# muzishen/IMAGHarmony

Hardware: AMD Instinct MI355X
Metric: 1024^2 SDXL images/sec (30 DDIM steps, PNS N seeds) (higher is better)
Workload: dtype bf16

## Files before the change

### imagharmony_amd/csrc/api.hip

```cpp
#include <stdarg.h>
#include <stdio.h>
#include <string.h>

#include <vector>

#include "../../include/imh.h"
#include "imh_common.h"
#include "imh_kernels.h"

namespace imh {

static thread_local char g_err[512] = "";

void set_error(const char* fmt, ...) {
    va_list ap;
    va_start(ap, fmt);
    vsnprintf(g_err, sizeof(g_err), fmt, ap);
    va_end(ap);
}

int experimental_refused(const char* what) {
    set_error("%s is compiled only with -DIMH_EXPERIMENTAL (IMH_EXPERIMENTAL=1 python -m imagharmony_amd.build): measured, not selected by any "
              "tuning.json entry or default mode", what);
    return IMH_ERR_ARG;
// ... 11 lines not shown
    GemmParams p;
    p.X = a->X; p.W = a->W; p.Y = a->Y; p.partial = a->partial; p.bias = a->bias; p.rowadd = a->rowadd;
    p.residual = a->residual; p.ln_s = a->ln_s; p.ln_c = a->ln_c; p.ln_eps = a->ln_eps;
    p.ln_stats = a->ln_stats; p.ln_stats_out = a->ln_stats_out; p.ln_slots = a->ln_slots; p.ln_slots_out = a->ln_slots_out;
    p.gn_out = a->gn_out; p.gn_nblk = a->gn_nblk; p.gn_hw = a->gn_hw;
    p.gn_tab = a->gn_tab; p.gn_silu = a->gn_silu; p.X2 = a->X2; p.Cin1 = a->X2 ? a->Cin1 : a->Cin;
    p.gn_src.partial = a->gn_part; p.gn_src.partial2 = a->gn_part2; p.gn_src.gamma = a->gn_gamma; p.gn_src.beta = a->gn_beta;
    p.gn_src.eps = a->gn_eps; p.gn_src.groups = a->gn_groups; p.gn_src.C = a->Cin; p.gn_src.C1 = a->gn_part2 ? a->gn_pC1 : a->Cin;
    p.gn_src.HW = a->H * a->Wd; p.gn_src.nblk = a->gn_pnblk; p.gn_src.sub = a->gn_psub; p.gn_src.npart = a->gn_pnpart;
    p.gn_src.nblk2 = a->gn_pnblk2; p.gn_src.sub2 = a->gn_psub2; p.gn_src.npart2 = a->gn_pnpart2; p.gn_src.dtype_f16 = a->dtype == IMH_DT_F16;
    p.Yt = a->Yt; p.yt_col0 = a->yt_col0; p.ldyt = a->ldyt;
    p.M = a->M; p.N = a->N; p.K = a->K;
    p.ldx = a->ldx; p.ldw = a->ldw; p.ldy = a->ldy; p.ldr = a->ldr; p.ldra = a->ldra > 0 ? a->ldra : a->N;
    p.rows_per_batch = a->rows_per_batch; p.splits = a->splits; p.flags = a->flags;
    p.H = a->H; p.Wd = a->Wd; p.Cin = a->Cin; p.Ho = a->Ho; p.Wo = a->Wo; p.stride = a->stride; p.up = a->up; p.pad_lo = a->pad == 1 ? 0 : 1;
    p.px = p.py = 1; p.tmx = p.tny = 0; p.xcd = a->xcd;
    p.pf_ptr = a->pf_ptr; p.pf_bytes = a->pf_bytes;
    p.early_res = g_ws_early;
    return p;
}

static int do_gemm_dual(const imh_gemm_args* a, const imh_gemm_args* b, hipStream_t s) {
    if (!a || !b || !a->X || !a->W || !a->Y || !b->X || !b->W || !b->Y) { set_error("gemm_dual: null pointer argument"); return IMH_ERR_ARG; }
    if (a->conv || b->conv || a->dtype != b->dtype) { set_error("gemm_dual: both problems must be plain GEMMs of one dtype"); return IMH_ERR_ARG; }
    int bm = a->bm, bn = a->bn;
    if (bm != 24128 && (bm <= 0 || bn <= 0 || bm > 128)) { bm = 128; bn = 64; }
    for (const imh_gemm_args* g : {a, b}) {
        if ((g->flags & (IMH_GF_LN_ROW | IMH_GF_LN_COL)) && (!g->ln_s || !g->ln_c || !(g->ln_eps > 0.f))) {
            set_error("gemm_dual: folded LayerNorm needs ln_s / ln_c / ln_eps > 0"); return IMH_ERR_ARG;
        }
// ... 12 lines not shown
    if ((p.flags & (IMH_GF_LN_ROW | IMH_GF_LN_COL)) && (!p.ln_s || !p.ln_c || !(p.ln_eps > 0.f))) { set_error("gemm: folded LayerNorm needs ln_s / ln_c / ln_eps > 0"); return IMH_ERR_ARG; }
    if ((p.flags & IMH_GF_LN_ROW) && (p.flags & IMH_GF_LN_COL)) { set_error("gemm: IMH_GF_LN_ROW and IMH_GF_LN_COL are exclusive"); return IMH_ERR_ARG; }
    if (!(p.flags & (IMH_GF_LN_ROW | IMH_GF_LN_COL))) p.ln_stats = nullptr;
    if (p.ln_stats && (p.ln_slots <= 0 || p.K % p.ln_slots)) { set_error("gemm: ln_slots=%d must divide K=%d", p.ln_slots, p.K); return IMH_ERR_ARG; }
    int bm = a->bm, bn = a->bn;
    if (bm <= 0 || bn <= 0 || p.splits <= 0) {
        int hb, hn, hs;
        gemm_pick_config(p.M, p.N, p.K, &hb, &hn, &hs);
        if (bm <= 0) bm = hb;
        if (bn <= 0) bn = hn;
        if (p.splits <= 0) p.splits = p.partial ? hs : 1;
    }
    if ((p.flags & IMH_GF_VT_PERM) && p.splits == 1) bn = 128;
    if (a->conv) {
        if (p.stride != 1 && p.stride != 2) { set_error("conv3x3: stride must be 1 or 2"); return IMH_ERR_ARG; }
        if (p.up != 0 && p.up != 1) { set_error("conv3x3: up must be 0 or 1"); return IMH_ERR_ARG; }
        if (a->pad != 0 && a->pad != 1) { set_error("conv3x3: pad must be 0 or 1"); return IMH_ERR_ARG; }
        if (a->pad == 1) {
            if (p.stride != 2 || p.up || p.H < 2 || p.Wd < 2) {
                set_error("conv3x3: pad mode 1 needs stride 2, up 0 and an input of at least 2 x 2 (stride=%d up=%d H=%d W=%d)", p.stride, p.up, p.H, p.Wd);
                return IMH_ERR_ARG;
            }
            if (bm == 7128 || bm == 7564 || bm == 7328 || bm == 7428 || bm == 7256 || bm == 7356 || bm == 8256 || bm == 9128 || bm == 9256 ||
                bm == 26256) {
                set_error("conv3x3: pad mode 1 is not implemented by variant %d x %d", bm, bn);
                return IMH_ERR_ARG;
            }
        }
        const int Hv = p.H << p.up, Wv = p.Wd << p.up;
        const int span = a->pad == 1 ? 1 : 2;
        if (p.Ho != (Hv + span - 3) / p.stride + 1 || p.Wo != (Wv + span - 3) / p.stride + 1 || p.Ho <= 0 || p.Wo <= 0) {
            set_error("conv3x3: output size %dx%d inconsistent with input %dx%d up=%d stride=%d pad=%d", p.Ho, p.Wo, p.H, p.Wd, p.up, p.stride, a->pad);
// ... 138 lines not shown
    if (key == 0) { g_attn_force_nw = value; return IMH_OK; }
    if (key == 1) {
#ifdef IMH_EXPERIMENTAL
        return 1;
#else
        return 0;
#endif
    }
    if (key == 2) { g_xcd_mode = value; return IMH_OK; }
    if (key == 3) { g_xattn_mode = value; return IMH_OK; }
    if (key == 4) { g_attn_mode = value; return IMH_OK; }
    if (key == 5) { g_halo_mode = value; return IMH_OK; }
    if (key == 7) { g_w16_pf = value; return IMH_OK; }
    if (key == 9) { g_w16_form = value; return IMH_OK; }
    if (key == 10) { g_f32_exact = value; return IMH_OK; }
    if (key == 6) { g_ws_early = value; return IMH_OK; }
    set_error("debug_set: unknown key %d", key);
    return IMH_ERR_ARG;
}
const char* imh_last_error(void) { return g_err; }

int imh_gemm(const imh_gemm_args* a, void* stream) { return do_gemm(a, (hipStream_t)stream); }
int imh_gemm_dual(const imh_gemm_args* a, const imh_gemm_args* b, void* stream) { return do_gemm_dual(a, b, (hipStream_t)stream); }
int imh_gemm_pick_config(int M, int N, int K, int* bm, int* bn, int* splits) {
    if (!bm || !bn || !splits) { set_error("pick_config: null output"); return IMH_ERR_ARG; }
    gemm_pick_config(M, N, K, bm, bn, splits);
    return IMH_OK;
}
size_t imh_gemm_workspace_bytes(int M, int N, int splits) { return gemm_workspace_bytes(M, N, splits); }
int imh_gemm_stats_slot_width(int bm, int bn) { return gemm_stats_slot_width(bm, bn); }
// ... 118 lines not shown
```

### imagharmony_amd/csrc/gemm.hip

```cpp
#include "imh_common.h"
#include "imh_kernels.h"
#include "imh_gemm_epilogue.h"
#include <algorithm>
#include <type_traits>

namespace imh {

int g_xcd_mode = 0;


template <typename T, int BM, int BN, bool CONV, int LN>
__device__ __forceinline__ void gemm_body(const GemmParams& p, const int bid, const int z) {
    constexpr int FM = BM / 32;
    constexpr int FN = BN / 32;
    constexpr int RX = BM / 32;
    constexpr int RW = BN / 32;
    constexpr int XT_BYTES = BM * GEMM_ROW_BYTES;
    constexpr int WT_BYTES = BN * GEMM_ROW_BYTES;
    constexpr int STAGE = XT_BYTES + WT_BYTES;
    typedef typename Vec<T>::v8 v8;

    extern __shared__ __attribute__((aligned(16))) unsigned char smem[];

    const int tid = threadIdx.x;
// ... 375 lines not shown
int gemm_gn_block_rows(int bm, int bn) {
    if ((bm == 1464 || bm == 2464) && bn == 160) return 32;
    if ((bm == 24128 || bm == 23256 || bm == 22128) && bn == 160) return 64;
    if (bm == 7128 || bm == 7328 || bm == 7428) return 32;
    if (bm == 7564) return 16;
    if (bm == 7256 || bm == 7356) return 64;
    return 0;
}

size_t gemm_workspace_bytes(int M, int N, int splits) {
    return splits > 1 ? (size_t)splits * M * N * sizeof(float) : 0;
}

int gemm_launch(GemmParams p, int dtype, int conv, int bm, int bn, hipStream_t stream) {
    if (p.K % GEMM_BK != 0 || p.K <= 0) { set_error("gemm: K=%d must be a positive multiple of 64", p.K); return IMH_ERR_SHAPE; }
    if (conv && (p.Cin % GEMM_BK != 0 || p.K != 9 * p.Cin)) { set_error("conv3x3: Cin=%d must be a multiple of 64 and K=9*Cin", p.Cin); return IMH_ERR_SHAPE; }
    if (!conv && ((p.ldx & 7) || (p.ldw & 7))) { set_error("gemm: ldx/ldw must be multiples of 8 elements"); return IMH_ERR_SHAPE; }
    if (p.M <= 0 || p.N <= 0) { set_error("gemm: empty problem M=%d N=%d", p.M, p.N); return IMH_ERR_SHAPE; }
    if ((p.flags & GF_GEGLU) && (p.N & 15)) { set_error("geglu: N must be a multiple of 16"); return IMH_ERR_SHAPE; }
    if (p.splits < 1) p.splits = 1;
    if (p.splits > 1 && !p.partial) { set_error("gemm: split-K needs a workspace"); return IMH_ERR_WORKSPACE; }
    if (p.rowadd && p.rows_per_batch <= 0) { set_error("gemm: rowadd needs rows_per_batch"); return IMH_ERR_ARG; }
    if ((p.flags & (GF_LN_ROW | GF_LN_COL)) && !p.ln_stats) {
        set_error("gemm: the folded LayerNorm takes the token rows' statistics from ln_stats (imh_lnstats.h: the epilogue of the GEMM that "
                  "wrote the rows, or IMH_EW_ROW_STATS); there is no in-loop E[x^2] - mean^2 form");
        return IMH_ERR_ARG;
    }
    if ((p.flags & (GF_LN_ROW | GF_LN_COL)) && (p.splits > 1 || (bm >= 256 && !((bm == 1464 || bm == 2464 || bm == 24128 || bm == 23256 || bm == 22128 || bm == 26256) && (p.flags & GF_LN_ROW))) || conv)) {
        set_error("gemm: folded LayerNorm needs a plain 64/128 tile or a wave-specialised variant (row form), splits == 1, no conv (bm=%d splits=%d conv=%d)", bm, p.splits, conv);
        return IMH_ERR_ARG;
    }
    if (p.ln_stats_out) {
        const int w = gemm_stats_slot_width(bm, bn);
        if (w == 0 || p.N % w || p.ln_slots_out != p.N / w || conv || p.splits > 1 || (p.flags & (GF_GEGLU | GF_VT_PERM | GF_OUT_F32))) {
            set_error("gemm: ln_stats_out needs a variant with a statistics epilogue (slot width %d for %dx%d), N %% width == 0, "
                      "ln_slots_out == N / width, a plain output (N=%d slots=%d flags=%d splits=%d conv=%d)", w, bm, bn, p.N, p.ln_slots_out, p.flags, p.splits, conv);
            return IMH_ERR_ARG;
        }
    }
    if (p.gn_out) {
        const int rows = gemm_gn_block_rows(bm, bn);
        const bool halo = bm >= 7000 && bm < 8000;
        if (rows == 0 || p.N % 10 || p.N % (halo ? bn : 80) || p.gn_hw <= 0 || p.gn_hw % rows || p.M % p.gn_hw || p.gn_nblk != p.gn_hw / rows ||
            p.splits > 1 || (p.flags & (GF_GEGLU | GF_VT_PERM | GF_OUT_F32 | GF_LN_ROW | GF_LN_COL)) ||
            (halo && (p.Ho % (rows * 4 / 16) || p.Wo % 16))) {
            set_error("gemm: gn_out needs a variant with a GroupNorm epilogue (%d rows per block for %dx%d), N a multiple of 10 and of the tile "
                      "width, whole tiles, gn_nblk == gn_hw / rows (N=%d hw=%d nblk=%d M=%d flags=%d)", rows, bm, bn, p.N, p.gn_hw, p.gn_nblk, p.M, p.flags);
            return IMH_ERR_ARG;
        }
    }
    {
        const bool halo = bm >= 7000 && bm < 8000;
        const bool ws = bm == 1464 || bm == 2464 || bm == 24128 || bm == 23256 || bm == 22128;
        if ((p.gn_tab || p.gn_src.partial) && !(conv && halo)) {
            set_error("gemm: the fused GroupNorm front end (gn_tab / gn_part) is a form of the LDS-halo conv3x3 (variant %d)", bm);
            return IMH_ERR_ARG;
        }
        if (p.gn_src.partial && (p.gn_tab || !gn_src_ok(p.gn_src))) {
// ... 33 lines not shown
```

### imagharmony_amd/csrc/gemm_ring.hip

```cpp
#include "imh_common.h"
#include "imh_kernels.h"
#include "imh_gemm_epilogue.h"
#include "imh_lnstats.h"
#include <type_traits>

namespace imh {

int g_ws_early = 1;

template <int N> __device__ __forceinline__ void wait_vmcnt() {
    asm volatile("s_waitcnt vmcnt(%0)" ::"n"(N) : "memory");
}

template <typename T, int BM, int BN, int WM, int WN, int S, bool CONV>
__global__ __launch_bounds__(64 * WM * WN, 1) void gemm_ring_kernel(const GemmParams p) {
    constexpr int NW = WM * WN;
    constexpr int NT = 64 * NW;
    constexpr int TM = BM / WM, TN = BN / WN;
    constexpr int FM = TM / 16, FN = TN / 16;
    constexpr int RPR = NW * 8;
    constexpr int RX = BM / RPR, RW = BN / RPR;
    constexpr int LP = RX + RW;
    constexpr int XT_BYTES = BM * GEMM_ROW_BYTES;
    constexpr int WT_BYTES = BN * GEMM_ROW_BYTES;
// ... 7 lines not shown

    const int tid = threadIdx.x;
    const int lane = tid & 63;
    const int wave = __builtin_amdgcn_readfirstlane(tid >> 6);
    const int wm = wave / WN, wn = wave % WN;

    int m0, n0;
    if (!xcd_tile<BM, BN>(p, blockIdx.x, m0, n0)) return;

    const int nkt = p.K / GEMM_BK;
    const int z = blockIdx.y;
    const int per = (nkt + p.splits - 1) / p.splits;
    const int kt0 = z * per;
    const int kt1 = min(nkt, kt0 + per);
    const int nt = max(0, kt1 - kt0);

    const unsigned char* zero = g_zero_page;
    const int srow = wave * 8 + (lane >> 3);

    const unsigned char* xbase[RX];
    int xstep[RX];
    int cb[RX], coy[RX], cox[RX];
    bool cvalid[RX];
#pragma unroll
    for (int i = 0; i < RX; ++i) {
        const int row = i * RPR + srow;
        const int c = stage_chunk_x(row, lane);
        const int m = m0 + row;
        const bool ok = m < p.M;
        if (!CONV) {
// ... 16 lines not shown
        const int row = i * RPR + srow;
        const int c = stage_chunk_w(row, lane, FN);
        const int n = n0 + row;
        const bool ok = n < p.N;
        wbase[i] = ok ? (const unsigned char*)p.W + ((size_t)n * p.ldw) * sizeof(T) + c * 16 : zero + c * 16;
        wstep[i] = ok ? GEMM_BK * (int)sizeof(T) : 0;
    }
    const int cpt = CONV ? p.Cin / GEMM_BK : 1;

    auto stage = [&](int slot, int kt) {
        unsigned char* xs = smem + slot * STAGE;
        unsigned char* ws = xs + XT_BYTES;
        if (CONV) {
            const int tap = kt / cpt;
            const int ct = kt - tap * cpt;
            const int ky = tap / 3, kx = tap - ky * 3;
            const int Hv = p.H << p.up, Wv = p.Wd << p.up;
#pragma unroll
            for (int i = 0; i < RX; ++i) {
                const int c = stage_chunk_x(i * RPR + srow, lane);
                const int iy = coy[i] * p.stride + ky - p.pad_lo;
                const int ix = cox[i] * p.stride + kx - p.pad_lo;
                const bool ok = cvalid[i] && iy >= 0 && iy < Hv && ix >= 0 && ix < Wv;
                const size_t pix = ((size_t)cb[i] * p.H + (iy >> p.up)) * p.Wd + (ix >> p.up);
                const unsigned char* src = ok
                    ? (const unsigned char*)p.X + (pix * p.Cin + (size_t)ct * GEMM_BK) * sizeof(T) + c * 16
                    : zero + c * 16;
                glds16(src, xs + (i * RPR + wave * 8) * GEMM_ROW_BYTES);
            }
        } else {
#pragma unroll
// ... 60 lines not shown
        if (m >= p.M || nb >= p.N) continue;
        float v[4 * FN];
#pragma unroll
        for (int j = 0; j < FN; ++j)
#pragma unroll
            for (int r = 0; r < 4; ++r) v[j * 4 + r] = acc[i][j][r];
        if (p.splits > 1) {
            float* o = p.partial + ((size_t)z * p.M + m) * p.N + nb;
            if (nb + 4 * FN <= p.N && (p.N & 3) == 0) {
#pragma unroll
                for (int q0 = 0; q0 < 4 * FN; q0 += 4) *(f32x4*)(o + q0) = f32x4{v[q0], v[q0 + 1], v[q0 + 2], v[q0 + 3]};
            } else {
#pragma unroll
                for (int q = 0; q < 4 * FN; ++q) if (nb + q < p.N) o[q] = v[q];
            }
        } else {
            epilogue_store<T, FN>(p, v, m, nb);
        }
    }
    if (z == 0) tail_prefetch(p.pf_ptr, p.pf_bytes, blockIdx.x, gridDim.x, tid, blockDim.x);
}

template <typename T, int BM, int BN, bool CONV>
__global__ __launch_bounds__(512, 2) void gemm_kg2_kernel(const GemmParams p) {
    constexpr int FM = BM / 32, FN = BN / 32;
    constexpr int RX = BM / 32, RW = BN / 32;
    constexpr int XT_BYTES = BM * GEMM_ROW_BYTES;
    constexpr int WT_BYTES = BN * GEMM_ROW_BYTES;
    constexpr int STAGE = XT_BYTES + WT_BYTES;
    constexpr int GROUP_BYTES = 2 * STAGE;
// ... 198 lines not shown
    const int tid = threadIdx.x;
    const int lane = tid & 63;
    const int wave = __builtin_amdgcn_readfirstlane(tid >> 6);

#if WS_TIMING
    const unsigned long long ts_entry = __builtin_amdgcn_s_memrealtime();
#endif
    int m0, n0;
    if (!xcd_tile<BM, BN>(p, bid, m0, n0)) return;
    const int nkt = p.K / GEMM_BK;
    const int z = blockIdx.y;
    const int per = (nkt + p.splits - 1) / p.splits;
    const int kt0 = z * per;
    const int kt1 = min(nkt, kt0 + per);
    const int nt = max(0, kt1 - kt0);

    if (wave >= NC) {
        const int pw = wave - NC;
        const unsigned char* zero = g_zero_page;
        const unsigned char* base[LP];
        const unsigned char* base2[KX > 0 ? KX : 1];
        const int kt_x2 = (!CONV && p.X2) ? p.Cin1 / GEMM_BK : 0x7fffffff;
        int step[LP];
        int cb[KX > 0 ? KX : 1], coy[KX > 0 ? KX : 1], cox[KX > 0 ? KX : 1];
        bool cvalid[KX > 0 ? KX : 1];
#pragma unroll
        for (int k = 0; k < LP; ++k) {
            const int r = (k * NL + pw) * 8 + (lane >> 3);
            if (k < KX) {
                const int c = stage_chunk_x(r, lane);
// ... 18 lines not shown
                const int c = stage_chunk_w(row, lane, FN);
                const int n = n0 + row;
                const bool ok = n < p.N;
                base[k] = ok ? (const unsigned char*)p.W + ((size_t)n * p.ldw) * sizeof(T) + c * 16 : zero + c * 16;
                step[k] = ok ? GEMM_BK * (int)sizeof(T) : 0;
            }
        }
        const int cpt = CONV ? p.Cin / GEMM_BK : 1;
        auto issue = [&](int slot, int kt) {
            unsigned char* st = smem + slot * STAGE;
            int ky = 0, kx = 0, ct = 0;
            if (CONV) {
                const int tap = kt / cpt;
                ct = kt - tap * cpt;
                ky = tap / 3; kx = tap - ky * 3;
            }
#pragma unroll
            for (int k = 0; k < LP; ++k) {
                unsigned char* dst = st + (k * NL + pw) * 8 * GEMM_ROW_BYTES;
                if (CONV && k < KX) {
                    const int r = (k * NL + pw) * 8 + (lane >> 3);
                    const int c = stage_chunk_x(r, lane);
                    const int Hv = p.H << p.up, Wv = p.Wd << p.up;
                    const int iy = coy[k] * p.stride + ky - p.pad_lo;
                    const int ix = cox[k] * p.stride + kx - p.pad_lo;
                    const bool ok = cvalid[k] && iy >= 0 && iy < Hv && ix >= 0 && ix < Wv;
                    const size_t pix = ((size_t)cb[k] * p.H + (iy >> p.up)) * p.Wd + (ix >> p.up);
                    const unsigned char* src = ok
                        ? (const unsigned char*)p.X + (pix * p.Cin + (size_t)ct * GEMM_BK) * sizeof(T) + c * 16
                        : zero + c * 16;
// ... 141 lines not shown
    }
    if (nt > 0) mm(K1);
#if WS_TIMING
    const unsigned long long ts_loop1 = __builtin_amdgcn_s_memrealtime();
    if (bid == 0 && wave == 0 && lane == 0 && p.pf_ptr) {
        unsigned long long* dbg = (unsigned long long*)p.pf_ptr;
        dbg[0] = tacc[0]; dbg[1] = tacc[1]; dbg[2] = tacc[2]; dbg[3] = nt;
    }
    if (wave == 0 && lane == 0 && p.pf_ptr && p.pf_bytes == 0xfeed) {
        unsigned long long* dbg = (unsigned long long*)p.pf_ptr + 8 + (size_t)bid * 4;
        dbg[0] = ts_entry; dbg[1] = ts_loop0; dbg[2] = ts_loop1; dbg[3] = 0;
    }
#endif

    const int nb = n0 + wn * TN + (lane >> 4) * 4 * FN;
    float lnpre[8 * FN];
    const bool have_pre = ln_preload<4 * FN>(p, nb, lnpre);
    EpiPre<4 * FN> pre;
    pre.ok = !p.rowadd && !p.residual && p.splits == 1 && epilogue_fast<T, 4 * FN>(p, nb);
    if (pre.ok && p.bias) ldv<T, 4 * FN>((const T*)p.bias + nb, pre.bias);
    LnArgs<4 * FN> ln;
    float st_s[FM], st_q[FM];
    constexpr int GNV = (4 * FN) % 10 == 0 ? 4 * FN : 10;
    GnAcc<GNV> gna;
    gn_zero(gna);
    if constexpr (LN == 2) {
        const f32x2s* ex = (const f32x2s*)(smem + S * STAGE);
#pragma unroll
        for (int q = 0; q < 4 * FN; ++q) {
            const f32x2s mr = ex[wn * TN + (lane >> 4) * 4 * FN + q];
            ln.cm[q] = mr[0]; ln.cr[q] = mr[1];
        }
    }
    if constexpr (LN == 1) {
        const float* ex = (const float*)(smem + S * STAGE);
// ... 158 lines not shown
#pragma unroll
        for (int j = 0; j < FN; ++j)
#pragma unroll
            for (int r = 0; r < 4; ++r) v[j * 4 + r] = acc[i][j][r];
        if (p.splits > 1) {
            float* o = p.partial + ((size_t)z * p.M + m) * p.N + nb;
            if (nb + 4 * FN <= p.N && (p.N & 3) == 0) {
#pragma unroll
                for (int q0 = 0; q0 < 4 * FN; q0 += 4) *(f32x4*)(o + q0) = f32x4{v[q0], v[q0 + 1], v[q0 + 2], v[q0 + 3]};
            } else {
#pragma unroll
                for (int q = 0; q < 4 * FN; ++q) if (nb + q < p.N) o[q] = v[q];
            }
        } else {
            if constexpr (LN == 1) { ln.mean = st_s[i]; ln.rstd = st_q[i]; }
            epilogue_store_pre<T, FN>(p, v, m, nb, lnpre, have_pre, LN != 0 ? &ln : nullptr, LN != 0 ? nullptr : &pre, lane,
                                      (LN == 0 && (4 * FN) % 10 == 0) ? &gna : nullptr, i == 0);
        }
    }
    if constexpr (LN == 0 && (4 * FN) % 10 == 0) {
        if (p.gn_out && p.splits == 1) {
            const int mw = m0 + wm * TM;
            if (mw < p.M) gn_emit<4 * FN>(p.gn_out, p.gn_nblk, p.N / 10, mw / p.gn_hw, (mw % p.gn_hw) / TM, nb, gna, FM, lane);
        }
    }
}

template <typename T, int BM, int BN, int CM, int CN, int S, int NP, bool CONV, int LN, int OCC = 1>
__global__ __launch_bounds__(64 * (CM * CN + NP), OCC == 1 ? 1 : OCC * (CM * CN + NP) / 4) void gemm_ws_kernel(const GemmParams p) {
    extern __shared__ __attribute__((aligned(16))) unsigned char smem[];
    gemm_ws_body<T, BM, BN, CM, CN, S, NP, CONV, LN>(p, blockIdx.x, gridDim.x, smem);
#if WS_TIMING
    if (threadIdx.x == 0 && p.pf_ptr && p.pf_bytes == 0xfeed) {
        asm volatile("s_waitcnt vmcnt(0)" ::: "memory");
        ((unsigned long long*)p.pf_ptr)[8 + (size_t)blockIdx.x * 4 + 3] = __builtin_amdgcn_s_memrealtime();
    }
#endif
}
// ... 124 lines not shown
```

### imagharmony_amd/csrc/imh_gemm_epilogue.h

```cpp
#pragma once
#include "imh_common.h"
#include "imh_kernels.h"
#include "imh_lnstats.h"

namespace imh {

template <int BM, int BN>
__device__ __forceinline__ bool xcd_tile(const GemmParams& p, int b, int& m0, int& n0) {
    if (p.px == 0) {
        m0 = (b / p.tny) * BM;
        n0 = (b % p.tny) * BN;
        return m0 < p.M;
    }
    const int xcd = b & 7, s = b >> 3;
    const int xi = xcd / p.py, yi = xcd - xi * p.py;
    const int ms = s / p.tny, ns = s - ms * p.tny;
    m0 = (xi * p.tmx + ms) * BM;
    n0 = (yi * p.tny + ns) * BN;
    return ms < p.tmx && m0 < p.M && n0 < p.N;
}

inline void xcd_partition(GemmParams& p, int bm, int bn, int* grid) {
    const int tm = (p.M + bm - 1) / bm, tn = (p.N + bn - 1) / bn;
    if (g_xcd_mode == 1) { p.px = 0; p.py = 1; p.tmx = tm; p.tny = tn; *grid = tm * tn; return; }
    int bpx = 8, bpy = 1;
    double best = 1e300;
    const int cand[4][2] = {{8, 1}, {4, 2}, {2, 4}, {1, 8}};
    for (auto& c : cand) {
        const int tmx = (tm + c[0] - 1) / c[0], tny = (tn + c[1] - 1) / c[1];
        const double waste = (double)(tmx * c[0]) * (tny * c[1]) / ((double)tm * tn);
        const double cost = ((double)c[1] * p.M + (double)c[0] * p.N) * waste * waste;
        if (cost < best) { best = cost; bpx = c[0]; bpy = c[1]; }
    }
    const int forced = g_xcd_mode ? g_xcd_mode : p.xcd;
    if (forced >= 2 && forced <= 5) { bpx = cand[forced - 2][0]; bpy = cand[forced - 2][1]; }
    p.px = bpx; p.py = bpy;
    p.tmx = (tm + bpx - 1) / bpx;
    p.tny = (tn + bpy - 1) / bpy;
    *grid = 8 * p.tmx * p.tny;
}

enum : int {
    GF_GEGLU = 1,
    GF_ACT_GELU = 2,
    GF_ACT_SILU = 4,
    GF_VT_PERM = 8,
    GF_OUT_F32 = 16,
    GF_LN_ROW = 32,
    GF_LN_COL = 64,
};

template <typename T, int CNT>
__device__ __forceinline__ void ldv(const T* p, float* o) {
    static_assert(CNT % 2 == 0, "vector epilogue works on even column counts");
// ... 243 lines not shown
```

### imagharmony_amd/csrc/imh_kernels.h

```cpp
#pragma once
#include <hip/hip_runtime.h>
#include <stddef.h>
#include "imh_gntable.h"

namespace imh {

struct GemmParams {
    const void* X;
    const void* W;
    void* Y;
    float* partial;
    const void* bias;
    const void* rowadd;
    const void* residual;
    const float* ln_s;
    const float* ln_c;
    float ln_eps;
    const float* ln_stats;
    float* ln_stats_out;
    int ln_slots, ln_slots_out;
    float* gn_out;
    int gn_nblk, gn_hw;
    const float* gn_tab;
    int gn_silu;
    GnTabSrc gn_src;
    const void* X2;
    int Cin1;
    void* Yt;
    int yt_col0, ldyt;
    int M, N, K;
    int ldx, ldw, ldy, ldr, ldra;
    int rows_per_batch;
    int splits;
    int flags;
    int H, Wd, Cin, Ho, Wo, stride, up, pad_lo;
    int px, py, tmx, tny;
    int xcd;
    const void* pf_ptr;
    unsigned pf_bytes;
    int early_res;
};

void gemm_pick_config(int M, int N, int K, int* bm, int* bn, int* splits);
size_t gemm_workspace_bytes(int M, int N, int splits);
int gemm_stats_slot_width(int bm, int bn);
int gemm_gn_block_rows(int bm, int bn);
int gemm_launch(GemmParams p, int dtype, int conv, int bm, int bn, hipStream_t stream);
int gemm_dual_launch(GemmParams a, GemmParams b, int dtype, int bm, int bn, hipStream_t stream);
int gemm_w16_launch(const GemmParams& p, int dtype, hipStream_t stream);

// ... 29 lines not shown
    const float* ln_stats;
    int ln_slots;
    int C, ldx, ldw;
    int split;
};
int xattn_launch(const XAttnParams& p, int dtype, hipStream_t stream);
extern int g_attn_force_nw;
extern int g_xattn_mode;
extern int g_w16_pf;
extern int g_w16_form;
extern int g_f32_exact;
extern int g_attn_mode;
extern int g_xcd_mode;
extern int g_halo_mode;
extern int g_ws_early;

struct SmallAttnParams {
    const void* Q; const void* K; const void* V; void* O;
    int B, H, Lq, Lk, dq, dv;
    int ldq, ldk, ldv, ldo;
    float scale;
};
int attention_small_launch(const SmallAttnParams& p, int dtype, hipStream_t stream);

struct NormParams {
    const void* x;
    void* y;
    const void* gamma;
    const void* beta;
    float* partial;
// ... 51 lines not shown
```

### imagharmony_amd/ctx.py

```python
import ctypes as C
import json
import os

import torch

from . import lib as L

_DT = {torch.bfloat16: L.IMH_DT_BF16, torch.float16: L.IMH_DT_F16}
_TUNING_PATH = os.environ.get("IMH_TUNING_PATH") or os.path.join(os.path.dirname(os.path.abspath(__file__)), "tuning.json")


_TUNING_CACHE = None


def _load_tuning():
    global _TUNING_CACHE
    if _TUNING_CACHE is None:
        _TUNING_CACHE = _read_tuning()
    return _TUNING_CACHE


def _read_tuning():
    try:
        with open(_TUNING_PATH) as f:
            raw = json.load(f)
        extra = os.environ.get("IMH_TUNING_OVERRIDE")
        if extra:
            raw.update(json.loads(extra))
        return {tuple(int(v) for v in k.split(",")): tuple(cfg) for k, cfg in raw.items()}
    except (OSError, ValueError):
        return {}


class GnStats:
    __slots__ = ("t", "nblk", "sub", "npart", "C")

    def __init__(self, t, nblk, sub, npart, C_):
        self.t, self.nblk, self.sub, self.npart, self.C = t, int(nblk), int(sub), int(npart), int(C_)


class GnSpec:
    def __init__(self, stats, gamma, beta, groups, eps):
        self.srcs = list(stats) if isinstance(stats, (list, tuple)) else [stats]
        self.gamma, self.beta, self.groups, self.eps = gamma, beta, int(groups), float(eps)
        self.C = sum(g.C for g in self.srcs)

# ... 119 lines not shown
    def _p(t):
        return None if t is None else t.data_ptr()

    def _chk(self, t, name, dtype=None):
        if t is None:
            return
        if t.device != self.device and not (t.device.type == "cuda" and t.device.index == (self.device.index or 0)):
            raise L.ImhError(f"{name}: tensor on {t.device}, context on {self.device}")
        if t.dtype != (dtype or self.dtype):
            raise L.ImhError(f"{name}: dtype {t.dtype}, expected {dtype or self.dtype}")

    _WS = (1464, 2464, 24128, 23256, 22128)
    _W16 = (26256,)
    _PP = (8256, 9128, 9256)
    _HALO = (7128, 7564, 7328, 7428, 7256, 7356)

    @classmethod
    def _variant_ok(cls, bm, sp, flags, conv, stride, ln_pre, M=0, N=0, extras=False, pad=0):
        plain = bm <= 128
        if pad and (not conv or bm in cls._HALO + cls._PP + cls._W16):
            return False
        if bm in cls._W16:
            return not conv and sp == 1 and bool(flags & L.GF_LN_ROW) and not flags & ~(L.GF_LN_ROW | L.GF_GEGLU) and bool(ln_pre) \
                and not extras and M % 256 == 0 and N % 320 == 0
        if bm in cls._HALO:
            return bool(conv) and stride == 1 and not flags & (L.GF_LN_ROW | L.GF_LN_COL | L.GF_VT_PERM)
        if flags & (L.GF_VT_PERM | L.GF_LN_COL):
            return plain and (sp == 1 or not flags & L.GF_LN_COL)
        if flags & L.GF_LN_ROW:
            return sp == 1 and not conv and (plain or bm in cls._WS)
# ... 163 lines not shown
        else:
            L.check(self.lib.imh_gemm_dual(C.byref(pair[0]), C.byref(pair[1]), self.stream()), descr)
        if own is not None:
            self.free(own[0])
        return o1, o2

    def conv_fuses_gn(self, M, N, K, stride=1, up=0, cfg=None):
        bm, bn, sp = cfg or self._config(M, N, K, 1, 0, stride=stride, up=up)
        if bm not in self._HALO or stride != 1 or up:
            return False
        ph = 4 if bm == 7564 else (16 if bm in (7256, 7356) else 8)
        S = (6 if ph == 16 else 9) if bn == 80 else (3 if bm in (7328, 7356) else (4 if bm == 7428 else 2))
        lds = 2 * (((ph + 2) * 18 + 7) // 8) * 8 * 128 + S * bn * 128 + (K // 9) * 8
        return lds <= 160 * 1024

    def conv3x3(self, x, w, bias=None, stride=1, up=0, residual=None, rowadd=None, ldra=0, out=None, cfg=None,
                descr="conv3x3", gn_groups=0, gn=None, x2=None, pad=0):
        self._chk(x, descr + ".x"); self._chk(w, descr + ".w")
        B, H, W, C1 = x.shape
        Cin = C1 + (x2.shape[-1] if x2 is not None else 0)
        Cout = w.shape[0]
        Hv, Wv = H << up, W << up
        if pad and (stride != 2 or up or gn is not None or x2 is not None):
            raise L.ImhError(f"{descr}: pad mode 1 is a plain stride-2 conv (no upsampling, fused GroupNorm or second source)")
        Ho, Wo = ((Hv - 2) // 2 + 1, (Wv - 2) // 2 + 1) if pad else ((Hv - 1) // stride + 1, (Wv - 1) // stride + 1)
        M, N, K = B * Ho * Wo, Cout, 9 * Cin
        if not x.is_contiguous() or not w.is_contiguous() or w.shape[1] != K:
            raise L.ImhError(f"{descr}: x must be contiguous NHWC and w packed [Cout, 9*Cin]")
        if x2 is not None:
            self._chk(x2, descr + ".x2")
            if tuple(x2.shape[:3]) != (B, H, W) or not x2.is_contiguous() or C1 % 64 or x2.shape[-1] % 64:
                raise L.ImhError(f"{descr}: x2 must be contiguous NHWC over the same pixels, both channel counts multiples of 64")
# ... 411 lines not shown
```

### imagharmony_amd/lib.py

```python
import ctypes as C
import os

_HERE = os.path.dirname(os.path.abspath(__file__))
_EXP_PATH = os.path.join(_HERE, "..", "tools", "tmp_libs", "libimh_hip_experimental.so")
LIB_PATH = os.environ.get("IMH_LIB_PATH") or (_EXP_PATH if os.environ.get("IMH_EXPERIMENTAL") == "1" else os.path.join(_HERE, "libimh_hip.so"))

ABI_VERSION = 11
IMH_DT_BF16, IMH_DT_F16 = 0, 1
GF_GEGLU, GF_ACT_GELU, GF_ACT_SILU, GF_VT_PERM, GF_OUT_F32, GF_LN_ROW, GF_LN_COL = 1, 2, 4, 8, 16, 32, 64
OP_GEMM, OP_ATTN, OP_GROUPNORM, OP_LAYERNORM, OP_EW, OP_ATTN_SMALL, OP_GEMM_DUAL, OP_XATTN = 0, 1, 2, 3, 4, 5, 6, 7
GN_ALL, GN_STATS, GN_TABLE, GN_APPLY, GN_TABLE_APPLY = 0, 1, 2, 3, 4
(EW_TIMESTEP, EW_SILU, EW_CONCAT, EW_CONV_IN, EW_CFG_STEP, EW_CAST_F32, EW_ADD, EW_STEP_SET, EW_CFG_RESCALE, EW_SOFTMAX,
 EW_ROW_STATS, EW_STEP_ROW) = range(12)

EXP_VARIANTS = {(4064, 64), (4064, 128), (4128, 64), (5256, 320), (6128, 320), (6064, 160), (7064, 160), (256, 128), (256, 256), (22128, 160),
                (3128, 128), (24128, 128), (9256, 320), (7564, 320), (7564, 160), (7328, 160), (7428, 160), (7256, 80)}


def experimental():
    return load().imh_debug_set(1, 0) == 1


def variant_built(cfg):
    return (int(cfg[0]), int(cfg[1])) not in EXP_VARIANTS or experimental()
# ... 140 lines not shown
```

### imagharmony_amd/unet.py

```python
import math
import os
from dataclasses import dataclass
from typing import Dict, Tuple

import torch
import torch.nn as nn

from . import lib as L
from .attention_processor import AttnProcessor2_0, IPAttnProcessor2_0, _b, _vkey, _w
from .ctx import Ctx, GnSpec


FOLD_LAYERNORM = True
LN_STATS_HANDOVER = os.environ.get("IMH_LN_STATS", "1") != "0"
GN_STATS_HANDOVER = os.environ.get("IMH_GN_STATS", "1") != "0"
GN_FUSE = os.environ.get("IMH_GN_FUSE", "1") != "0"
GN_TABLE_FOLD = os.environ.get("IMH_GN_TABLE_FOLD", "1") != "0"


class Feat:
    __slots__ = ("t", "gs")

    def __init__(self, t, gs=None):
        self.t, self.gs = t, gs

    def stats(self, ctx, groups):
        if self.gs is None:
            B, C_ = self.t.shape[0], self.t.shape[-1]
            self.gs = ctx.gn_stats(self.t.view(B, -1, C_), sub=math.gcd(C_ // groups, 10))
        return self.gs
# ... 40 lines not shown


class Conv2d(nn.Module):
    def __init__(self, cin, cout, k):
        super().__init__()
        self.weight = nn.Parameter(torch.empty(cout, cin, k, k), requires_grad=False)
        self.bias = nn.Parameter(torch.empty(cout), requires_grad=False)

    def packed(self, ctx):
        key = (_vkey(self.weight), ctx.dtype, str(ctx.device))
        c = getattr(self, "_imh_packed", None)
        if c is None or c[0] != key:
            w = self.weight.detach().permute(0, 2, 3, 1).reshape(self.weight.shape[0], -1)
            c = (key, w.to(device=ctx.device, dtype=ctx.dtype).contiguous())
            self._imh_packed = c
        return c[1]


class Norm(nn.Module):
    def __init__(self, c, eps):
        super().__init__()
        self.weight = nn.Parameter(torch.empty(c), requires_grad=False)
        self.bias = nn.Parameter(torch.empty(c), requires_grad=False)
        self.eps = eps


class Dropout(nn.Module):
    pass


# ... 567 lines not shown
        h = mb.resnets[0].emit(ctx, h, st, keep_input=True)
        ctx.tag = 31
        h = mb.attentions[0].emit(ctx, h, kv_of(mb.attentions[0]), st)
        ctx.tag = 30
        h = mb.resnets[1].emit(ctx, h, st)
        for bi, blk in enumerate(self.up_blocks):
            for i, r in enumerate(blk.resnets):
                ctx.tag = 40 + bi
                h = r.emit(ctx, h, st, skip=skips.pop())
                if blk.has_attn:
                    ctx.tag = 50 + bi
                    h = blk.attentions[i].emit(ctx, h, kv_of(blk.attentions[i]), st)
            if blk.upsamplers is not None:
                ctx.tag = 40 + bi
                u = blk.upsamplers[0].conv
                r_ = ctx.conv3x3(h.t, u.packed(ctx), bias=_b(u, ctx), up=1, descr="upsample", gn_groups=1 if ho else 0)
                h.free(ctx)
                h = Feat(*r_) if ho else Feat(r_)
        ctx.tag = 60
        Bh, Hh, Ww, C0 = h.t.shape
        if GN_TABLE_FOLD:
            n = ctx.gn_table_apply(h.t.view(B, Hh * Ww, C0), GnSpec(h.stats(ctx, cfg.norm_num_groups), _w(self.conv_norm_out, ctx), _b(self.conv_norm_out, ctx),
                                                                    cfg.norm_num_groups, cfg.norm_eps), True, descr="conv_norm_out").view(B, Hh, Ww, C0)
        else:
            tab = ctx.gn_table(h.stats(ctx, cfg.norm_num_groups), _w(self.conv_norm_out, ctx), _b(self.conv_norm_out, ctx), cfg.norm_num_groups, cfg.norm_eps,
                               Hh * Ww, descr="conv_norm_out.table")
            n = ctx.gn_apply(h.t.view(B, Hh * Ww, C0), tab, True, descr="conv_norm_out").view(B, Hh, Ww, C0)
            ctx.free(tab)
        h.free(ctx)
        out = ctx.conv3x3(n, self.conv_out.packed(ctx), bias=_b(self.conv_out, ctx), descr="conv_out")
        ctx.free(n)
# ... 33 lines not shown
```

### include/imh.h

```cpp
#ifndef IMH_H_
#define IMH_H_

#include <stddef.h>
#include <stdint.h>

#ifdef __cplusplus
extern "C" {
#endif

#define IMH_ABI_VERSION 11

enum imh_status {
    IMH_OK = 0,
    IMH_ERR_ARG = -1,
    IMH_ERR_SHAPE = -2,
    IMH_ERR_DTYPE = -3,
    IMH_ERR_LAUNCH = -4,
    IMH_ERR_WORKSPACE = -5
};

enum imh_dtype { IMH_DT_BF16 = 0, IMH_DT_F16 = 1 };

enum imh_gemm_flags {
    IMH_GF_GEGLU = 1,
    IMH_GF_ACT_GELU = 2,
// ... 241 lines not shown
```

Baseline: 1.689.

## Compute nearest-upsample + 3x3 conv as four 2x2 phase convolutions

Replaces the upsampler's nearest-2x upsample followed by a 3x3 convolution with an equivalent sub-pixel (phase) form. The weights are pre-summed into four 2x2 kernels, one per output phase, and run as a single GEMM over low-resolution pixels with K = 4*Cin instead of 9*Cin. Output rows are scattered to interleaved high-resolution positions, and the GroupNorm statistics epilogue is adapted to the per-phase blocks. This cuts the upsample conv FLOPs by roughly 4/9 and avoids reading the virtual upsampled input. In exchange it adds weight-packing code and constrains which tile variants can be used, and summing the weights changes rounding slightly.

After: 1.709 (median of 6 runs). 1.01x the previous value.

```diff
diff --git a/imagharmony_amd/csrc/api.hip b/imagharmony_amd/csrc/api.hip
--- a/imagharmony_amd/csrc/api.hip
+++ b/imagharmony_amd/csrc/api.hip
@@ -49,6 +49,7 @@
     p.ldx = a->ldx; p.ldw = a->ldw; p.ldy = a->ldy; p.ldr = a->ldr; p.ldra = a->ldra > 0 ? a->ldra : a->N;
     p.rows_per_batch = a->rows_per_batch; p.splits = a->splits; p.flags = a->flags;
     p.H = a->H; p.Wd = a->Wd; p.Cin = a->Cin; p.Ho = a->Ho; p.Wo = a->Wo; p.stride = a->stride; p.up = a->up; p.pad_lo = a->pad == 1 ? 0 : 1;
+    p.phase = 0; p.pN = 0;
     p.px = p.py = 1; p.tmx = p.tny = 0; p.xcd = a->xcd;
     p.pf_ptr = a->pf_ptr; p.pf_bytes = a->pf_bytes;
     p.early_res = g_ws_early;
@@ -91,8 +92,19 @@
     if ((p.flags & IMH_GF_VT_PERM) && p.splits == 1) bn = 128;
     if (a->conv) {
         if (p.stride != 1 && p.stride != 2) { set_error("conv3x3: stride must be 1 or 2"); return IMH_ERR_ARG; }
-        if (p.up != 0 && p.up != 1) { set_error("conv3x3: up must be 0 or 1"); return IMH_ERR_ARG; }
+        if (p.up != 0 && p.up != 1 && p.up != 2) { set_error("conv3x3: up must be 0, 1 or 2"); return IMH_ERR_ARG; }
         if (a->pad != 0 && a->pad != 1) { set_error("conv3x3: pad must be 0 or 1"); return IMH_ERR_ARG; }
+        if (p.up == 2) {
+            if (!g_up_phase) { set_error("conv3x3: the phase form (up = 2) is switched off (imh_debug_set key 11)"); return IMH_ERR_ARG; }
+            if (p.stride != 1 || a->pad != 0 || p.H <= 0 || p.Wd <= 0 || p.Ho != 2 * p.H || p.Wo != 2 * p.Wd || p.M % (p.H * p.Wd) != 0 ||
+                p.N <= 0 || p.N % 4 || p.K != 4 * p.Cin) {
+                set_error("conv3x3: the phase form (up = 2) needs stride 1, pad 0, Ho x Wo = 2H x 2W, M = B*H*W low-res pixels, N = 4*Cout, "
+                          "K = 4*Cin (H=%d W=%d Ho=%d Wo=%d M=%d N=%d K=%d Cin=%d stride=%d)", p.H, p.Wd, p.Ho, p.Wo, p.M, p.N, p.K, p.Cin, p.stride);
+                return IMH_ERR_SHAPE;
+            }
+            p.phase = 1; p.pN = p.N / 4; p.up = 0; p.Ho = p.H; p.Wo = p.Wd;
+            return gemm_launch(p, a->dtype, a->conv, bm, bn, s);
+        }
         if (a->pad == 1) {
             if (p.stride != 2 || p.up || p.H < 2 || p.Wd < 2) {
                 set_error("conv3x3: pad mode 1 needs stride 2, up 0 and an input of at least 2 x 2 (stride=%d up=%d H=%d W=%d)", p.stride, p.up, p.H, p.Wd);
@@ -261,6 +273,7 @@
     if (key == 7) { g_w16_pf = value; return IMH_OK; }
     if (key == 9) { g_w16_form = value; return IMH_OK; }
     if (key == 10) { g_f32_exact = value; return IMH_OK; }
+    if (key == 11) { if (value >= 0) g_up_phase = value; return g_up_phase; }
     if (key == 6) { g_ws_early = value; return IMH_OK; }
     set_error("debug_set: unknown key %d", key);
     return IMH_ERR_ARG;
diff --git a/imagharmony_amd/csrc/gemm.hip b/imagharmony_amd/csrc/gemm.hip
--- a/imagharmony_amd/csrc/gemm.hip
+++ b/imagharmony_amd/csrc/gemm.hip
@@ -413,7 +413,18 @@
 
 int gemm_launch(GemmParams p, int dtype, int conv, int bm, int bn, hipStream_t stream) {
     if (p.K % GEMM_BK != 0 || p.K <= 0) { set_error("gemm: K=%d must be a positive multiple of 64", p.K); return IMH_ERR_SHAPE; }
-    if (conv && (p.Cin % GEMM_BK != 0 || p.K != 9 * p.Cin)) { set_error("conv3x3: Cin=%d must be a multiple of 64 and K=9*Cin", p.Cin); return IMH_ERR_SHAPE; }
+    if (conv && (p.Cin % GEMM_BK != 0 || p.K != (p.phase ? 4 : 9) * p.Cin)) { set_error("conv3x3: Cin=%d must be a multiple of 64 and K=9*Cin (phase form: 4*Cin)", p.Cin); return IMH_ERR_SHAPE; }
+    if (p.phase) {
+        const bool ws = bm == 1464 || bm == 2464 || bm == 24128 || bm == 23256;
+        const bool okv = (ws && bn == 160) || (bm == 23256 && bn == 128) || (bm == 5258 && bn == 320);
+        if (!conv || !okv || p.pN <= 0 || p.pN % bn || (p.pN & 7) || p.N != 4 * p.pN || p.splits > 1 || p.flags || p.residual || p.rowadd || p.X2 ||
+            p.ln_stats_out || p.gn_tab || p.gn_src.partial || p.Yt || p.ldy != p.pN || p.stride != 1 || p.pad_lo != 1 || p.up) {
+            set_error("conv3x3: the phase form (up = 2) needs a wave-specialised bn = 160 variant, 23256 x 128 or 5258 x 320, Cout a multiple of bn, "
+                      "ldy == Cout, bias as the only epilogue input, no split-K (bm=%d bn=%d Cout=%d N=%d ldy=%d splits=%d flags=%d)",
+                      bm, bn, p.pN, p.N, p.ldy, p.splits, p.flags);
+            return IMH_ERR_ARG;
+        }
+    }
     if (!conv && ((p.ldx & 7) || (p.ldw & 7))) { set_error("gemm: ldx/ldw must be multiples of 8 elements"); return IMH_ERR_SHAPE; }
     if (p.M <= 0 || p.N <= 0) { set_error("gemm: empty problem M=%d N=%d", p.M, p.N); return IMH_ERR_SHAPE; }
     if ((p.flags & GF_GEGLU) && (p.N & 15)) { set_error("geglu: N must be a multiple of 16"); return IMH_ERR_SHAPE; }
@@ -440,7 +451,8 @@
     if (p.gn_out) {
         const int rows = gemm_gn_block_rows(bm, bn);
         const bool halo = bm >= 7000 && bm < 8000;
-        if (rows == 0 || p.N % 10 || p.N % (halo ? bn : 80) || p.gn_hw <= 0 || p.gn_hw % rows || p.M % p.gn_hw || p.gn_nblk != p.gn_hw / rows ||
+        const int cout = p.phase ? p.pN : p.N;
+        if (rows == 0 || cout % 10 || cout % (halo ? bn : 80) || p.gn_hw <= 0 || p.gn_hw % rows || p.M % p.gn_hw || p.gn_nblk != (p.phase ? 4 : 1) * (p.gn_hw / rows) ||
             p.splits > 1 || (p.flags & (GF_GEGLU | GF_VT_PERM | GF_OUT_F32 | GF_LN_ROW | GF_LN_COL)) ||
             (halo && (p.Ho % (rows * 4 / 16) || p.Wo % 16))) {
             set_error("gemm: gn_out needs a variant with a GroupNorm epilogue (%d rows per block for %dx%d), N a multiple of 10 and of the tile "
diff --git a/imagharmony_amd/csrc/gemm_ring.hip b/imagharmony_amd/csrc/gemm_ring.hip
--- a/imagharmony_amd/csrc/gemm_ring.hip
+++ b/imagharmony_amd/csrc/gemm_ring.hip
@@ -6,6 +6,7 @@
 
 namespace imh {
 
+int g_up_phase = 1;
 int g_ws_early = 1;
 
 template <int N> __device__ __forceinline__ void wait_vmcnt() {
@@ -45,6 +46,7 @@
     const int kt0 = z * per;
     const int kt1 = min(nkt, kt0 + per);
     const int nt = max(0, kt1 - kt0);
+    const int ph = (CONV && p.phase) ? n0 / p.pN : 0;
 
     const unsigned char* zero = g_zero_page;
     const int srow = wave * 8 + (lane >> 3);
@@ -91,7 +93,8 @@
         if (CONV) {
             const int tap = kt / cpt;
             const int ct = kt - tap * cpt;
-            const int ky = tap / 3, kx = tap - ky * 3;
+            int ky = tap / 3, kx = tap - ky * 3;
+            if (p.phase) { ky = (tap >> 1) + (ph >> 1); kx = (tap & 1) + (ph & 1); }
             const int Hv = p.H << p.up, Wv = p.Wd << p.up;
 #pragma unroll
             for (int i = 0; i < RX; ++i) {
@@ -182,6 +185,8 @@
 #pragma unroll
                 for (int q = 0; q < 4 * FN; ++q) if (nb + q < p.N) o[q] = v[q];
             }
+        } else if (CONV && p.phase) {
+            epilogue_store<T, FN>(p, v, phase_row(p, m, ph), nb - ph * p.pN);
         } else {
             epilogue_store<T, FN>(p, v, m, nb);
         }
@@ -410,6 +415,7 @@
     const int kt0 = z * per;
     const int kt1 = min(nkt, kt0 + per);
     const int nt = max(0, kt1 - kt0);
+    const int ph = (CONV && p.phase) ? n0 / p.pN : 0;
 
     if (wave >= NC) {
         const int pw = wave - NC;
@@ -458,6 +464,7 @@
                 const int tap = kt / cpt;
                 ct = kt - tap * cpt;
                 ky = tap / 3; kx = tap - ky * 3;
+                if (p.phase) { ky = (tap >> 1) + (ph >> 1); kx = (tap & 1) + (ph & 1); }
             }
 #pragma unroll
             for (int k = 0; k < LP; ++k) {
@@ -629,11 +636,12 @@
 #endif
 
     const int nb = n0 + wn * TN + (lane >> 4) * 4 * FN;
+    const int nbo = nb - ph * (CONV ? p.pN : 0);
     float lnpre[8 * FN];
     const bool have_pre = ln_preload<4 * FN>(p, nb, lnpre);
     EpiPre<4 * FN> pre;
-    pre.ok = !p.rowadd && !p.residual && p.splits == 1 && epilogue_fast<T, 4 * FN>(p, nb);
-    if (pre.ok && p.bias) ldv<T, 4 * FN>((const T*)p.bias + nb, pre.bias);
+    pre.ok = !p.rowadd && !p.residual && p.splits == 1 && epilogue_fast<T, 4 * FN>(p, nbo);
+    if (pre.ok && p.bias) ldv<T, 4 * FN>((const T*)p.bias + nbo, pre.bias);
     LnArgs<4 * FN> ln;
     float st_s[FM], st_q[FM];
     constexpr int GNV = (4 * FN) % 10 == 0 ? 4 * FN : 10;
@@ -822,14 +830,16 @@
             }
         } else {
             if constexpr (LN == 1) { ln.mean = st_s[i]; ln.rstd = st_q[i]; }
-            epilogue_store_pre<T, FN>(p, v, m, nb, lnpre, have_pre, LN != 0 ? &ln : nullptr, LN != 0 ? nullptr : &pre, lane,
+            const int mo = (CONV && p.phase) ? phase_row(p, m, ph) : m;
+            epilogue_store_pre<T, FN>(p, v, mo, nbo, lnpre, have_pre, LN != 0 ? &ln : nullptr, LN != 0 ? nullptr : &pre, lane,
                                       (LN == 0 && (4 * FN) % 10 == 0) ? &gna : nullptr, i == 0);
         }
     }
     if constexpr (LN == 0 && (4 * FN) % 10 == 0) {
         if (p.gn_out && p.splits == 1) {
             const int mw = m0 + wm * TM;
-            if (mw < p.M) gn_emit<4 * FN>(p.gn_out, p.gn_nblk, p.N / 10, mw / p.gn_hw, (mw % p.gn_hw) / TM, nb, gna, FM, lane);
+            const int nsub = ((CONV && p.phase) ? p.pN : p.N) / 10;
+            if (mw < p.M) gn_emit<4 * FN>(p.gn_out, p.gn_nblk, nsub, mw / p.gn_hw, ph * (p.gn_hw / TM) + (mw % p.gn_hw) / TM, nbo, gna, FM, lane);
         }
     }
 }
diff --git a/imagharmony_amd/csrc/imh_gemm_epilogue.h b/imagharmony_amd/csrc/imh_gemm_epilogue.h
--- a/imagharmony_amd/csrc/imh_gemm_epilogue.h
+++ b/imagharmony_amd/csrc/imh_gemm_epilogue.h
@@ -38,6 +38,15 @@
     p.tmx = (tm + bpx - 1) / bpx;
     p.tny = (tn + bpy - 1) / bpy;
     *grid = 8 * p.tmx * p.tny;
+}
+
+__device__ __forceinline__ int phase_row(const GemmParams& p, const int m, const int ph) {
+    const int hw = p.H * p.Wd;
+    const int b = m / hw;
+    const int rem = m - b * hw;
+    const int y = rem / p.Wd;
+    const int x = rem - y * p.Wd;
+    return ((b * 2 * p.H + 2 * y + (ph >> 1)) * 2 * p.Wd) + 2 * x + (ph & 1);
 }
 
 enum : int {
diff --git a/imagharmony_amd/csrc/imh_kernels.h b/imagharmony_amd/csrc/imh_kernels.h
--- a/imagharmony_amd/csrc/imh_kernels.h
+++ b/imagharmony_amd/csrc/imh_kernels.h
@@ -34,6 +34,7 @@
     int splits;
     int flags;
     int H, Wd, Cin, Ho, Wo, stride, up, pad_lo;
+    int phase, pN;
     int px, py, tmx, tny;
     int xcd;
     const void* pf_ptr;
@@ -93,6 +94,7 @@
 extern int g_xcd_mode;
 extern int g_halo_mode;
 extern int g_ws_early;
+extern int g_up_phase;
 
 struct SmallAttnParams {
     const void* Q; const void* K; const void* V; void* O;
diff --git a/imagharmony_amd/ctx.py b/imagharmony_amd/ctx.py
--- a/imagharmony_amd/ctx.py
+++ b/imagharmony_amd/ctx.py
@@ -30,6 +30,25 @@
         return {tuple(int(v) for v in k.split(",")): tuple(cfg) for k, cfg in raw.items()}
     except (OSError, ValueError):
         return {}
+
+
+_PHASE_TAPS = (((0,), (1, 2)), ((0, 1), (2,)))
+
+
+def phase_pack(w4):
+    w4 = w4.detach().float()
+    Cout, Cin = w4.shape[:2]
+    out = w4.new_empty(4, Cout, 2, 2, Cin)
+    for py in range(2):
+        for px in range(2):
+            for a in range(2):
+                for b in range(2):
+                    acc = None
+                    for ky in _PHASE_TAPS[py][a]:
+                        for kx in _PHASE_TAPS[px][b]:
+                            acc = w4[:, :, ky, kx] if acc is None else acc + w4[:, :, ky, kx]
+                    out[2 * py + px, :, a, b, :] = acc
+    return out.reshape(4 * Cout, 4 * Cin)
 
 
 class GnStats:
@@ -179,6 +198,8 @@
     _W16 = (26256,)
     _PP = (8256, 9128, 9256)
     _HALO = (7128, 7564, 7328, 7428, 7256, 7356)
+
+    _PHASE = ((1464, 160), (2464, 160), (24128, 160), (23256, 160), (23256, 128), (5258, 320))
 
     @classmethod
     def _variant_ok(cls, bm, sp, flags, conv, stride, ln_pre, M=0, N=0, extras=False, pad=0):
@@ -372,8 +393,64 @@
         lds = 2 * (((ph + 2) * 18 + 7) // 8) * 8 * 128 + S * bn * 128 + (K // 9) * 8
         return lds <= 160 * 1024
 
+    def conv_up_phase_cfg(self, B, H, W, Cin, Cout, cfg=None):
+        if Cin % 64 or Cout % 8 or min(B, H, W) < 1 or self.lib.imh_debug_set(11, -1) != 1:
+            return None
+        c = cfg or self.tuning.get((B * H * W, 4 * Cout, 4 * Cin, 1, 4)) or ((23256, 160, 1) if Cout % 160 == 0 else (23256, 128, 1))
+        bm, bn, sp = c
+        if (bm, bn) not in self._PHASE or Cout % bn or sp != 1:
+            return None
+        return bm, bn, 1
+
+    def _conv3x3_phase(self, x, w, w_phase, bias, out, cfg, descr, gn_groups):
+        B, H, W, Cin = x.shape
+        if w_phase is None:
+            self._chk(w, descr + ".w")
+            if w.dim() != 2 or w.shape[1] != 9 * Cin:
+                raise L.ImhError(f"{descr}: w must be packed [Cout, 9*Cin]")
+            w_phase = phase_pack(w.view(w.shape[0], 3, 3, Cin).permute(0, 3, 1, 2)).to(self.dtype).contiguous()
+        self._chk(x, descr + ".x"); self._chk(w_phase, descr + ".w_phase")
+        Cout = w_phase.shape[0] // 4
+        if not x.is_contiguous() or not w_phase.is_contiguous() or tuple(w_phase.shape) != (4 * Cout, 4 * Cin):
+            raise L.ImhError(f"{descr}: x must be contiguous NHWC and w_phase [4*Cout, 4*Cin]")
+        c = self.conv_up_phase_cfg(B, H, W, Cin, Cout, cfg=cfg)
+        if c is None:
+            raise L.ImhError(f"{descr}: the phase form (up=2) does not run this launch (Cin {Cin} % 64, Cout {Cout} % tile width, variant "
+                             f"{cfg}, imh_debug_set key 11); use up=1 (Ctx.conv_up_phase_cfg)")
+        bm, bn, sp = c
+        Ho, Wo = 2 * H, 2 * W
+        M, N, K = B * H * W, 4 * Cout, 4 * Cin
+        if out is None:
+            out = self.new(B, Ho, Wo, Cout)
+        a = L.GemmArgs()
+        a.X, a.W, a.Y, a.bias = x.data_ptr(), w_phase.data_ptr(), out.data_ptr(), self._p(bias)
+        a.M, a.N, a.K = M, N, K
+        a.ldx, a.ldw, a.ldy = Cin, K, Cout
+        a.rows_per_batch = H * W
+        a.splits, a.flags, a.dtype, a.conv, a.bm, a.bn = 1, 0, self.dt, 1, bm, bn
+        a.xcd = self._xcd_for(N, 0, 1)
+        a.H, a.Wd, a.Cin, a.Ho, a.Wo, a.stride, a.up, a.pad = H, W, Cin, Ho, Wo, 1, 2, 0
+        gs = None
+        rows = self.lib.imh_gemm_gn_block_rows(bm, bn)
+        if gn_groups and rows > 0 and Cout % 80 == 0 and (H * W) % rows == 0:
+            nblk = 4 * (H * W // rows)
+            t = self.new(B, nblk, Cout // 10, 2, dtype=torch.float32)
+            a.gn_out, a.gn_nblk, a.gn_hw = t.data_ptr(), nblk, H * W
+            gs = GnStats(t, nblk, 10, rows * 10, Cout)
+        es = x.element_size()
+        self._emit(L.OP_GEMM, a, descr=descr, flops=2.0 * (B * Ho * Wo) * Cout * 9 * Cin, nbytes=es * (M * Cin + N * K + 4 * M * Cout),
+                   keep=(x, w_phase, out, bias) + ((gs.t,) if gs else ()),
+                   shape=(B * Ho * Wo, Cout, 9 * Cin, 1, (B, H, W, Cin, 1, 2)),
+                   epi=dict(flags=0, bias=bias is not None, residual=False, rowadd=False, rows_per_batch=Ho * Wo, cfg=(bm, bn, sp),
+                            gn_out=(gs.nblk, Ho * Wo) if gs else None, gn_in=None, x2=0))
+        return (out, gs) if gn_groups else out
+
     def conv3x3(self, x, w, bias=None, stride=1, up=0, residual=None, rowadd=None, ldra=0, out=None, cfg=None,
-                descr="conv3x3", gn_groups=0, gn=None, x2=None, pad=0):
+                descr="conv3x3", gn_groups=0, gn=None, x2=None, pad=0, w_phase=None):
+        if up == 2:
+            if stride != 1 or pad or residual is not None or rowadd is not None or gn is not None or x2 is not None:
+                raise L.ImhError(f"{descr}: the phase form (up=2) is a plain stride-1 conv with a bias (no residual, row-add, fused GroupNorm or second source)")
+            return self._conv3x3_phase(x, w, w_phase, bias, out, cfg, descr, gn_groups)
         self._chk(x, descr + ".x"); self._chk(w, descr + ".w")
         B, H, W, C1 = x.shape
         Cin = C1 + (x2.shape[-1] if x2 is not None else 0)
diff --git a/imagharmony_amd/lib.py b/imagharmony_amd/lib.py
--- a/imagharmony_amd/lib.py
+++ b/imagharmony_amd/lib.py
@@ -5,7 +5,7 @@
 _EXP_PATH = os.path.join(_HERE, "..", "tools", "tmp_libs", "libimh_hip_experimental.so")
 LIB_PATH = os.environ.get("IMH_LIB_PATH") or (_EXP_PATH if os.environ.get("IMH_EXPERIMENTAL") == "1" else os.path.join(_HERE, "libimh_hip.so"))
 
-ABI_VERSION = 11
+ABI_VERSION = 12
 IMH_DT_BF16, IMH_DT_F16 = 0, 1
 GF_GEGLU, GF_ACT_GELU, GF_ACT_SILU, GF_VT_PERM, GF_OUT_F32, GF_LN_ROW, GF_LN_COL = 1, 2, 4, 8, 16, 32, 64
 OP_GEMM, OP_ATTN, OP_GROUPNORM, OP_LAYERNORM, OP_EW, OP_ATTN_SMALL, OP_GEMM_DUAL, OP_XATTN = 0, 1, 2, 3, 4, 5, 6, 7
diff --git a/imagharmony_amd/unet.py b/imagharmony_amd/unet.py
--- a/imagharmony_amd/unet.py
+++ b/imagharmony_amd/unet.py
@@ -14,6 +14,7 @@
 FOLD_LAYERNORM = True
 LN_STATS_HANDOVER = os.environ.get("IMH_LN_STATS", "1") != "0"
 GN_STATS_HANDOVER = os.environ.get("IMH_GN_STATS", "1") != "0"
+UPSAMPLE_PHASE = os.environ.get("IMH_UPSAMPLE_PHASE", "1") != "0"
 GN_FUSE = os.environ.get("IMH_GN_FUSE", "1") != "0"
 GN_TABLE_FOLD = os.environ.get("IMH_GN_TABLE_FOLD", "1") != "0"
 
@@ -84,6 +85,15 @@
             w = self.weight.detach().permute(0, 2, 3, 1).reshape(self.weight.shape[0], -1)
             c = (key, w.to(device=ctx.device, dtype=ctx.dtype).contiguous())
             self._imh_packed = c
+        return c[1]
+
+    def packed_phase(self, ctx):
+        from .ctx import phase_pack
+        key = (_vkey(self.weight), ctx.dtype, str(ctx.device))
+        c = getattr(self, "_imh_packed_phase", None)
+        if c is None or c[0] != key:
+            c = (key, phase_pack(self.weight).to(device=ctx.device, dtype=ctx.dtype).contiguous())
+            self._imh_packed_phase = c
         return c[1]
 
 
@@ -681,7 +691,11 @@
             if blk.upsamplers is not None:
                 ctx.tag = 40 + bi
                 u = blk.upsamplers[0].conv
-                r_ = ctx.conv3x3(h.t, u.packed(ctx), bias=_b(u, ctx), up=1, descr="upsample", gn_groups=1 if ho else 0)
+                Bu, Hu, Wu, Cu = h.t.shape
+                if UPSAMPLE_PHASE and ctx.conv_up_phase_cfg(Bu, Hu, Wu, Cu, u.weight.shape[0]) is not None:
+                    r_ = ctx.conv3x3(h.t, None, bias=_b(u, ctx), up=2, w_phase=u.packed_phase(ctx), descr="upsample", gn_groups=1 if ho else 0)
+                else:
+                    r_ = ctx.conv3x3(h.t, u.packed(ctx), bias=_b(u, ctx), up=1, descr="upsample", gn_groups=1 if ho else 0)
                 h.free(ctx)
                 h = Feat(*r_) if ho else Feat(r_)
         ctx.tag = 60
diff --git a/include/imh.h b/include/imh.h
--- a/include/imh.h
+++ b/include/imh.h
@@ -8,7 +8,7 @@
 extern "C" {
 #endif
 
-#define IMH_ABI_VERSION 11
+#define IMH_ABI_VERSION 12
 
 enum imh_status {
     IMH_OK = 0,
```
